# yzh503/vm-placement-migration-gym

Measured on AMD Instinct MI355X. Metric: env-steps/sec (batched) at 100-PM config, 1/2/4/8 GPUs; reward MAE vs CPU ref, higher is better.
Workload: dtype f64

## Files before the change

include/vmp.h:

```cpp
#ifndef VMP_H
#define VMP_H

#include <stdint.h>

#ifdef __cplusplus
extern "C" {
#endif

#define VMP_ABI_VERSION 14

#define VMP_OK 0
#define VMP_EINVAL (-1)
#define VMP_EDEVICE (-2)
#define VMP_EOOM (-3)
#define VMP_ESTATE (-4)

#define VMP_REWARD_WR 0
#define VMP_REWARD_UT 1
#define VMP_REWARD_KL 2
#define VMP_SEQ_UNIFORM 0
#define VMP_SEQ_LOWUNIFORM 1
#define VMP_SEQ_HIGHUNIFORM 2
#define VMP_REC_STEPS 0
#define VMP_REC_REWARD 1
// ... 196 lines not shown
int vmp_actor_head_bf16_sample(int32_t B, int32_t K, int32_t V, int32_t A, const uint16_t *h,
                               const uint16_t *weight, const float *bias,
                               const uint32_t *mask_bits, float wait_ratio, int32_t wait_index,
                               uint64_t seed, uint64_t offset, const uint64_t *rng_counter,
                               int32_t *action, float *logprob, float *entropy, float *workspace,
                               void *hip_stream);
int vmp_actor_head_bf16_bwd(int32_t B, int32_t K, int32_t V, int32_t A, const uint16_t *h,
                            const uint16_t *weight, const float *bias, const uint32_t *mask_bits,
                            const int32_t *action, const float *g_logprob,
                            const float *g_entropy, uint16_t *dlogits, int32_t ld, float *dbias,
                            float *workspace, void *hip_stream);
int64_t vmp_actor_head_bf16_bwd_workspace(int32_t B, int32_t V, int32_t A);

int vmp_record_enable(vmp_handle *h, int32_t on);
int vmp_record_read(vmp_handle *h, uint32_t *hist, double *sums);

int vmp_reqlog_enable(vmp_handle *h, int64_t capacity);
int vmp_reqlog_info(const vmp_handle *h, int64_t *capacity);
int vmp_reqlog_read(vmp_handle *h, int32_t *rows, int64_t *meta);

int vmp_series_enable(vmp_handle *h, int64_t capacity, int32_t stride, int32_t pm_rows);
int vmp_series_info(const vmp_handle *h, int64_t *capacity, int32_t *stride, int32_t *pm_rows);
int vmp_series_read(vmp_handle *h, double *rows, float *pm, int64_t *meta);

int vmp_debug_fail_alloc(int32_t n);
int64_t vmp_debug_live_allocs(void);

int vmp_debug_stamps(vmp_handle *h, uint64_t *out);

int vmp_debug_quiet_violations(int64_t *count);

int vmp_debug_occupancy(vmp_handle *h, int32_t *blocks_per_cu, int32_t *lds_bytes);

#ifdef __cplusplus
}
#endif
#endif
```

vm-placement-migration-gym_amd/csrc/vmp_capi.cpp:

```cpp
#include <hip/hip_runtime.h>

#include <cmath>
#include <cstdlib>
#include <cstring>
#include <string>
#include <vector>

#include "../../include/vmp.h"
#include "vmp_carve.h"
#include "vmp_host.h"
#include "vmp_kernels.h"
#include "vmp_layout.h"
#include "vmp_record.h"
#include "vmp_reqlog.h"
#include "vmp_series.h"
#include "vmp_trace.h"

using namespace vmp;

namespace vmp {
int policy_fail(int code, const char *msg) { return fail(code, msg); }
}

struct vmp_handle {
  vmp_config cfg;
  int32_t N, P, V, A, D, W32;
  int32_t device;
  int32_t eval_mode;
  hipStream_t stream;
  uint32_t *vmw;
  double *pm;
  EnvHdr *hdr;
  double *lg_arr, *lg_svc;
  PoisConst arr, svc;
  EnvParams prm;
  uint32_t *scratch_bits;
  PoisConst *pois_dev;
  uint64_t *stamps;
  uint64_t *jump_dev;
  uint8_t *bigscr;
  bool big;
  bool rec_on;
  RecArgs rec;
  int32_t *rec_act;
  uint8_t *rec_valid;
  double *rec_reward;
  bool rq_on;
  ReqArgs rq;
  bool sr_on;
  SerArgs sr;
  double *sr_reward;
  double *wl;
  PoisConst *wl_rec;
  PoisConst *pois_env;
  double *lg_shared;
  int32_t lg_shared_n;
  TraceDesc *tr_tab;
  uint64_t *tr_data;
  TraceDesc *tr_host;
  int32_t tr_n;
  int32_t *tr_map;
  int64_t *tr_info;
  uint64_t tr_hash;
};

namespace {

using EnvKernel = void (*)(EnvParams, StepOut);
template <int VPT>
EnvKernel env_kernel_tr(bool ext, bool one) {
  if (ext) return k_env_ext_tr<VPT>;
  return one ? k_env_tr<VPT, true> : k_env_tr<VPT, false>;
}
template <int VPT>
EnvKernel env_kernel(bool ext, bool one, bool wl, bool tr) {
  if (tr) return env_kernel_tr<VPT>(ext, one);
  if (ext) return wl ? k_env_ext<VPT, true> : k_env_ext<VPT, false>;
  if (one) return wl ? k_env<VPT, true, true> : k_env<VPT, true, false>;
  return wl ? k_env<VPT, false, true> : k_env<VPT, false, false>;
}

int launch_env(vmp_handle *h, const StepOut &o) {
  dim3 grid((h->N + kEnvWavesPerBlock - 1) / kEnvWavesPerBlock), block(64 * kEnvWavesPerBlock);
  EnvParams p = h->prm;
  const bool wl = h->pois_env != nullptr, tr = h->tr_tab != nullptr;
  const int spt = big_spt(h->V);
  p.scap = kSpecDraws;
  p.lds_wave_bytes = launch_wave_bytes(p, o.k_steps);
  const size_t lds = launch_lds(p, o.k_steps, h->big, spt);
  if (!lds_fits(lds, h->big)) return fail(VMP_EINVAL, "config too large for the LDS carve");
  if (h->big) {
    if (tr) launch_big_env_tr(spt, o.k_steps == 1, h->N, lds, h->stream, p, o);
    else if (wl) launch_big_env_wl(spt, o.k_steps == 1, h->N, lds, h->stream, p, o);
    else launch_big_env(spt, o.k_steps == 1, h->N, lds, h->stream, p, o);
    return launched();
  }
  if (o.actions && o.k_steps != 1) return fail(VMP_EINVAL, "external actions take one step per launch");
  const int need = (h->V + 63) / 64;
  const auto pick = need <= 1 ? env_kernel<1> : need <= 2 ? env_kernel<2> : need <= 4 ? env_kernel<4>
                    : need <= 8 ? env_kernel<8> : env_kernel<16>;
  hipLaunchKernelGGL(pick(o.actions != nullptr, o.k_steps == 1, wl, tr), grid, block, lds, h->stream, p, o);
  return launched();
}

StepOut empty_out() {
  StepOut o;
  std::memset(&o, 0, sizeof(o));
  o.policy = -1;
  return o;
}

void refresh_params(vmp_handle *h) {
  h->prm.eval_mode = h->eval_mode;
  h->prm.limit = h->eval_mode ? h->cfg.eval_steps : h->cfg.training_steps;
}

void scratch_free(vmp_handle *h) {
  dev_free(h->rec_act);
  dev_free(h->rec_valid);
  h->rec_act = nullptr;
  h->rec_valid = nullptr;
}

int record_init(vmp_handle *h, const uint8_t *env_mask) {
  size_t n = (size_t)h->N * h->V;
  if ((size_t)h->N * 2 * VMP_REC_BINS > n) n = (size_t)h->N * 2 * VMP_REC_BINS;
  if ((size_t)h->N * VMP_NREC > n) n = (size_t)h->N * VMP_NREC;
  hipLaunchKernelGGL(k_record_init, dim3((unsigned)((n + 255) / 256)), dim3(256), 0, h->stream,
                     h->prm, h->rec, env_mask);
  return launched();
// ... 59 lines not shown
    return fail(VMP_EINVAL, "vms must be in [1, 10240] on this build");
  if (cfg->reward_function < 0 || cfg->reward_function > 2)
    return fail(VMP_EINVAL, "Function does not exist: reward_function");
  if (cfg->sequence < 0 || cfg->sequence > 2) return fail(VMP_EINVAL, "unknown sequence");
  if (!(cfg->arrival_rate >= 0) || !(cfg->service_length >= 0))
    return fail(VMP_EINVAL, "arrival_rate and service_length must be >= 0");
  for (int32_t i = 0; i < n_env; i++)
    if (seeds[i] < 0) return fail(VMP_EINVAL, "seeds must be non-negative");
  HIP_TRY(hipSetDevice(device));
  vmp_handle *h = new vmp_handle();
  std::memset(h, 0, sizeof(*h));
  h->cfg = *cfg;
  h->N = n_env;
  h->P = cfg->pms;
  h->V = cfg->vms;
  h->A = cfg->allow_null_action ? cfg->pms + 2 : cfg->pms + 1;
  h->D = 3 * cfg->vms + 2 * cfg->pms;
  h->W32 = (h->A + 31) / 32;
  const char *force = getenv("VMP_BIG_KERNEL");
  h->big = cfg->vms > kMaxVPT * kWaveSize || (force && force[0] == '1');
  h->device = device;
  h->stream = nullptr;
  int rc = setup_pois(cfg->arrival_rate, h->arr, &h->lg_arr);
  if (rc == VMP_OK) rc = setup_pois(cfg->service_length, h->svc, &h->lg_svc);
  if (rc == VMP_OK) rc = create_rest(h, cfg, n_env, seeds);
  if (rc != VMP_OK) return fail_after(rc, [&] { vmp_destroy(h); });
  *out = h;
  return VMP_OK;
}

static int create_rest(vmp_handle *h, const vmp_config *cfg, int32_t n_env, const int64_t *seeds) {
  hipError_t e1 = dev_malloc(&h->vmw, sizeof(uint32_t) * (size_t)n_env * vm_pitch(h->V));
  hipError_t e2 = dev_malloc(&h->pm, sizeof(double) * (size_t)n_env * 2 * h->P);
  hipError_t e3 = dev_malloc(&h->hdr, sizeof(EnvHdr) * (size_t)n_env);
  if (e1 != hipSuccess || e2 != hipSuccess || e3 != hipSuccess)
    return fail(VMP_EOOM, "device allocation failed");
  HIP_TRY(hipMemset(h->hdr, 0, sizeof(EnvHdr) * (size_t)n_env));
  EnvParams &p = h->prm;
  p.N = h->N;
  p.P = h->P;
  p.V = h->V;
  p.A = h->A;
  p.D = h->D;
  p.W32 = h->W32;
  p.reward = cfg->reward_function;
  p.cap_target_util = cfg->cap_target_util;
  int64_t M = cfg->training_steps > cfg->eval_steps ? cfg->training_steps : cfg->eval_steps;
  p.M2 = 2 * M;
  p.beta = cfg->beta;
  p.seq_lo = cfg->sequence == VMP_SEQ_HIGHUNIFORM ? 0.25 : 0.1;
  double hi = cfg->sequence == VMP_SEQ_LOWUNIFORM ? 0.65 : 1.0;
  p.seq_range = hi - p.seq_lo;
  {
    PoisConst pc[2] = {h->arr, h->svc};
    HIP_TRY(dev_malloc(&h->pois_dev, sizeof(pc)));
    HIP_TRY(hipMemcpy(h->pois_dev, pc, sizeof(pc), hipMemcpyHostToDevice));
    p.pois = h->pois_dev;
    uint64_t jt[kJumpWords];
    pcg_jump_table(jt);
    HIP_TRY(dev_malloc(&h->jump_dev, sizeof(jt)));
    HIP_TRY(hipMemcpy(h->jump_dev, jt, sizeof(jt), hipMemcpyHostToDevice));
    p.jump = h->jump_dev;
  }
  p.vmw = h->vmw;
  p.pm = h->pm;
  p.hdr = h->hdr;
  if (h->big) carve_big(h->P, h->V, p);
  else carve_wave(h->P, h->V, p);
  if (h->big) {
    HIP_TRY(dev_malloc(&h->bigscr, (size_t)n_env * 4 * (size_t)h->V));
// ... 722 lines not shown
  SnapDesc d;
  HIP_TRY(hipStreamSynchronize(h->stream));
  HIP_TRY(hipMemcpy(&d, src, sizeof(d), hipMemcpyDeviceToHost));
  if (d.magic != kSnapMagic || d.abi != VMP_ABI_VERSION || d.hdr_bytes != (int32_t)sizeof(EnvHdr))
    return fail(VMP_EINVAL, "vmp_restore: not a snapshot of this library version");
  if (d.N != h->N || d.P != h->P || d.V != h->V || d.A != h->A || !same_config(d.cfg, h->cfg))
    return fail(VMP_EINVAL, "vmp_restore: snapshot of another env count or config");
  const uint8_t *s = (const uint8_t *)src;
  const SnapLayout l(h);
  if ((d.workload != 0) != (h->wl != nullptr))
    return fail(VMP_EINVAL, "vmp_restore: snapshot and handle differ in having a per-env workload");
  if ((d.traced != 0) != (h->tr_tab != nullptr))
    return fail(VMP_EINVAL, "vmp_restore: snapshot and handle differ in having a trace");
  if (h->tr_tab && d.trace_hash != h->tr_hash)
    return fail(VMP_EINVAL, "vmp_restore: snapshot of another trace");
  if (h->wl) {
    std::vector<double> w(2 * (size_t)h->N);
    HIP_TRY(hipMemcpy(w.data(), s + l.wl, l.nw, hipMemcpyDeviceToHost));
    if (std::memcmp(w.data(), h->wl, l.nw) != 0)
      return fail(VMP_EINVAL, "vmp_restore: snapshot of another per-env workload");
  }
  HIP_TRY(hipMemcpyAsync(h->hdr, s + l.hdr, l.nh, hipMemcpyDeviceToDevice, h->stream));
  HIP_TRY(hipMemcpyAsync(h->pm, s + l.pm, l.np, hipMemcpyDeviceToDevice, h->stream));
  HIP_TRY(hipMemcpyAsync(h->vmw, s + l.vmw, l.nv, hipMemcpyDeviceToDevice, h->stream));
  if (h->rec_on)
    if (const int rc = record_init(h, nullptr)) return rc;
  if (h->rq_on)
    if (const int rc = reqlog_init(h, nullptr)) return rc;
  return h->sr_on ? series_init(h, nullptr) : VMP_OK;
}

int64_t vmp_debug_live_allocs(void) { return g_live.load(); }

int vmp_debug_quiet_violations(int64_t *count) {
  if (!count) return fail(VMP_EINVAL, "null argument");
  const int64_t v = quiet_violations_take();
  if (v == -1) return fail(VMP_EINVAL, "library built without -DVMP_CHECK_QUIET");
  if (v < 0) return fail(VMP_EDEVICE, "vmp_debug_quiet_violations: device read failed");
  *count = v;
  return VMP_OK;
}

int vmp_debug_fail_alloc(int32_t n) {
  if (n < 0) return fail(VMP_EINVAL, "n must be >= 0");
  g_fail_alloc.store(n);
  return VMP_OK;
}

int vmp_debug_occupancy(vmp_handle *h, int32_t *blocks_per_cu, int32_t *lds_bytes) {
  if (!h || !blocks_per_cu || !lds_bytes) return fail(VMP_EINVAL, "null argument");
  if (!h->big) return fail(VMP_EINVAL, "occupancy query covers the block kernel (V > 1024) only");
  const int spt = big_spt(h->V);
  const size_t lds1 = launch_lds(h->prm, 1, true, spt);
  int st = 0;
  *blocks_per_cu = big_occupancy(spt, lds1, &st);
  *lds_bytes = (int32_t)lds1 + st;
  return VMP_OK;
}

int vmp_debug_stamps(vmp_handle *h, uint64_t *out) {
  if (!h || !out) return fail(VMP_EINVAL, "null argument");
  if (!h->stamps) return fail(VMP_EINVAL, "library built without -DVMP_STAMPS");
  HIP_TRY(hipMemcpyAsync(out, h->stamps, sizeof(uint64_t) * kStamps * (size_t)h->N,
                         hipMemcpyDeviceToDevice, h->stream));
  HIP_TRY(hipMemsetAsync(h->stamps, 0, sizeof(uint64_t) * kStamps * (size_t)h->N, h->stream));
  return VMP_OK;
// ... 4 lines not shown
```

vm-placement-migration-gym_amd/csrc/vmp_env_aux.h:

```cpp
#ifndef VMP_ENV_AUX_H
#define VMP_ENV_AUX_H

#include <hip/hip_runtime.h>
#include <stdint.h>

#include "vmp_dev.h"
#include "vmp_env_common.h"
#include "vmp_kernels.h"
#include "vmp_layout.h"
#include "vmp_np_rng.h"
#include "vmp_np_sum.h"

namespace vmp {

__global__ __launch_bounds__(256) void k_reset(EnvParams p, const int64_t *seeds,
                                               const uint8_t *env_mask, float *obs) {
  const int lane = lane_id();
  const int e = uni(blockIdx.x * kWavesPerBlock + (threadIdx.x >> 6));
  if (e >= p.N) return;
  if (env_mask && !env_mask[e]) return;
  EnvHdr *h = p.hdr + e;
  const int V = p.V, P = p.P;
  if (lane < 4) {
    Pcg r;
// ... 160 lines not shown
  __syncthreads();
  const int lane = lane_id(), e = blockIdx.x;
  const Lds L = make_lds(p, (char LDSP *)lds);
  const int V = p.V, P = p.P;
  const uint32_t *row = p.vmw + (int64_t)e * vm_pitch(V);
  int n_ex = 0;
  for (int b = 0; b < V; b += 64) {
    const int v = b + lane;
    const uint32_t w = v < V ? row[vm_slot_idx(v)] : (uint32_t)(P + 1);
    const bool ex = v < V && (int)(w & 0xFFFFu) <= P;
    const uint64_t m = ballot(ex);
    if (ex) {
      const int rk = n_ex + below(m, lane);
      L.ccomp[rk] = (uint8_t)((w >> 16) & 0xFFu);
      L.mcomp[rk] = (uint8_t)((w >> 24) & 0xFFu);
    }
    n_ex += __popcll(m);
  }
  wsync();
  const double *ct = cent;
  const uint8_t LDSP *cc = L.ccomp;
  const uint8_t LDSP *cm = L.mcomp;
  const double sc = wave_pw_sum(n_ex, [=](int i) { return ct[cc[i]]; }, L.pw);
  const double sm = wave_pw_sum(n_ex, [=](int i) { return ct[cm[i]]; }, L.pw);
  if (lane == 0) {
    double tcm = sc / (double)P, tmm = sm / (double)P;
    if (p.cap_target_util && tcm > 1) tcm = 1.0;
    if (p.cap_target_util && tmm > 1) tmm = 1.0;
    p.hdr[e].tcm = tcm;
    p.hdr[e].tmm = tmm;
  }
}

}

#endif
```

vm-placement-migration-gym_amd/csrc/vmp_env_wave.h:

```cpp
#ifndef VMP_ENV_WAVE_H
#define VMP_ENV_WAVE_H

#include <hip/hip_runtime.h>
#include <stdint.h>

#include "vmp_dev.h"
#include "vmp_env_common.h"
#include "vmp_kernels.h"
#include "vmp_layout.h"
#include "vmp_stamps.h"

namespace vmp {

template <int VPT>
__device__ __forceinline__ int64_t heuristic_apply(const EnvParams &p, const Lds &L,
                                                   const Tables &T, uint32_t (&wa)[VPT],
                                                   int policy, int32_t *act_out,
                                                   uint8_t *valid_out, bool quiet, int qkind,
                                                   bool &fit_any STAMP_PARAMS) {
  const int lane = lane_id();
  const int P = p.P, WAIT = p.P;
  const bool bf = policy == 1;
  uint32_t pend = 0;
#pragma unroll
  for (int s = 0; s < VPT; s++)
    if (w_pl(wa[s]) == WAIT) pend |= 1u << s;
  uint32_t won = 0, bad = 0;
  int64_t n_place = 0;
  fit_any = false;
#ifdef VMP_CHECK_QUIET
  if (ballot(pend != 0)) {
#else
  if (!quiet && ballot(pend != 0)) {
#endif
    for (int i = lane; i < P; i += 64) {
      const float fcv = (float)L.cpu[i], fmv = (float)L.mem[i];
      L.fcpu[i] = fcv;
      L.fmem[i] = fmv;
      L.tc[i] = (uint8_t)(fit_threshold(fcv) + 1);
      L.tm[i] = (uint8_t)(fit_threshold(fmv) + 1);
    }
// ... 422 lines not shown

template <int VPT>
__device__ __forceinline__ void write_mask(const EnvParams &p, const Lds &L, const Tables &T,
                                           const uint32_t (&wa)[VPT], uint32_t *bits) {
  const int lane = fresh_lane();
  const int P = p.P, A = p.A, W = p.W32, WAIT = p.P, NUL = p.P + 1;
#pragma unroll
  for (int s = 0; s < VPT; s++) {
    const int v = s * 64 + lane;
    const bool in = live(wa[s]);
    const int c = in ? w_pl(wa[s]) : NUL;
    const double vc = T.cent[w_cc(wa[s])], vm = T.cent[w_cm(wa[s])];
    const bool waiting = in && c == WAIT;
    const bool anyw = ballot(waiting) != 0;
#pragma unroll 1
    for (int w = 0; w < W; w++) {
      uint32_t word = 0xFFFFFFFFu;
      const int a0 = w * 32;
      if (c >= a0 && c < a0 + 32 && c < A) word &= ~(1u << (c - a0));
      if (c < P && WAIT >= a0 && WAIT < a0 + 32) word &= ~(1u << (WAIT - a0));
      if (anyw) {
        const int hi = min(a0 + 32, P);
#pragma unroll 1
        for (int q = a0; q < hi; q++) {
          const bool fit = (L.cpu[q] + vc <= 1) && (L.mem[q] + vm <= 1);
          if (waiting && fit) word &= ~(1u << (q - a0));
        }
      }
      if (in) bits[(int64_t)v * W + w] = word;
    }
  }
}

__device__ __forceinline__ bool idle_step(const EnvParams &p, const StepOut &o, const Lds &L) {
#ifdef VMP_CHECK_QUIET
  return false;
#else
  const uint64_t ph = L.hdr->pad;
  const uint32_t t32 = (uint32_t)L.hdr->timestep;
  const uint32_t nf = (uint32_t)ph;
  const bool q1 = (ph >> 62) & 1u, q2 = (ph >> 60) & 1u;
  const bool idle = o.k_steps == 1 && p.reward == 0 && !o.act_out && !o.valid && !o.mask_bits &&
                    2 * p.P <= 256 && (ph >> 63) && q1 != q2 &&
                    (ph & 0x0FFFFFFF00000000ull) == 0 && nf != 0u && (int32_t)(nf - t32) > 1;
  return uni((int)idle) != 0;
#endif
}

template <int VPT>
__device__ __forceinline__ void idle_body(const EnvParams &p, const StepOut &o, const Lds &L,
                                          const float LDSP *fcent, int e,
                                          const uint32_t (&wa)[VPT]) {
  const int lane = lane_id();
  const int V = p.V;
  EnvHdr LDSP *H = L.hdr;
  const int64_t a = L.arr[0];
  const uint64_t ph = H->pad;
  const int64_t ts = H->timestep;
  const bool term = ts >= p.limit;
  if (lane == 0) {
    if (o.reward) gptr(o.reward)[e] = ((ph >> 61) & 1u) ? -H->waiting_ratio : 0.0;
    if (o.done) gptr(o.done)[e] = (uint8_t)term;
    if (o.done_count) gptr(o.done_count)[e] += (int64_t)term;
  }
  if (o.obs) {
    float *obs = o.obs + (int64_t)e * p.D;
#pragma unroll
    for (int s = 0; s < VPT; s++) {
      const int v = s * 64 + lane;
      if (live(wa[s])) {
        ST_NT(obs + v, (float)w_pl(wa[s]));
        ST_NT(obs + V + v, fcent[w_cc(wa[s])]);
        ST_NT(obs + 2 * V + v, fcent[w_cm(wa[s])]);
      }
    }
    for (int i = lane; i < 2 * p.P; i += 64) ST_NT(obs + 3 * V + i, (float)L.cpu[i]);
  }
  wsync();
  if (lane == 0) {
    H->timestep = ts + 1;
    H->total_requests += a;
    H->dropped += a;
  }
  wsync();
  if (lane < 32)
    gptr(reinterpret_cast<uint64_t *>(p.hdr + e))[lane] = reinterpret_cast<uint64_t LDSP *>(H)[lane];
}

template <int VPT, bool ONE, bool EXT, int SRC>
__device__ __forceinline__ void env_body(const EnvParams &p, const StepOut &o) {
  extern __shared__ __align__(16) char lds[];
  __shared__ Tables T;
#ifdef VMP_STAMPS
  const uint64_t t_start = __builtin_amdgcn_s_memtime();
  const uint64_t rt_start = __builtin_amdgcn_s_memrealtime();
#endif
  const int lane = lane_id();
  const int wid = threadIdx.x >> 6;
  const int e_raw = uni(blockIdx.x * kEnvWavesPerBlock + wid);
  const int e = e_raw < p.N ? e_raw : p.N - 1;
  char LDSP *base = (char LDSP *)lds + wid * p.lds_wave_bytes;
  const Lds L = make_lds(p, base);
  const int V = p.V, P = p.P;
  __builtin_amdgcn_s_setprio(2);
  const uint64_t hv = gptr(reinterpret_cast<const uint64_t *>(p.hdr + e))[lane & 31];
  static_assert(kEnvWavesPerBlock == 1, "Tables::pois holds one env's Poisson constants");
  constexpr int kPoisWords = (int)(2 * sizeof(PoisConst) / 4);
  uint32_t pw = 0;
  if constexpr (SRC != kSrcTrace)
    pw = gptr(reinterpret_cast<const uint32_t *>(env_pois<SRC>(p, e)))[threadIdx.x % kPoisWords];
  TraceDesc td{nullptr, nullptr, 0, 0};
  if constexpr (SRC == kSrcTrace) td = env_trace(p, e);
  U128 JA{0, 0}, JM{0, 0};
  if (SRC != kSrcTrace && o.k_steps > 0) {
    const uint64_t GLBP *jt = gptr(p.jump + 4 * lane);
    JA = U128{jt[0], jt[1]};
    JM = U128{jt[2], jt[3]};
  }
  const double *pm = p.pm + (int64_t)e * 2 * P;
  const int n_pm = 2 * P;
  double pv[4];
#pragma unroll
  for (int j = 0; j < 4; j++) pv[j] = pm[min(j * 64 + lane, n_pm - 1)];
  __asm__ volatile("" ::: "memory");
  const uint32_t GLBP *vlo = gptr(p.vmw + (int64_t)e * vm_pitch(V));
  uint32_t wa[VPT], rem[VPT];
#pragma unroll
  for (int s = 0; s < VPT; s++) {
    const int v = s * 64 + lane;
    const uint32_t x = vlo[vw_row(s, lane)];
    wa[s] = v < V ? x : (uint32_t)kPad;
    if (ONE) {
      rem[s] = 0;
    } else {
      const uint32_t y = vlo[vw_row(s, lane) + 64];
      rem[s] = v < V ? y : 0u;
    }
  }
// ... 16 lines not shown
#pragma unroll
    for (int j = 0; j < 4; j++)
      if (j * 64 + lane < n_pm) L.cpu[j * 64 + lane] = pv[j];
  }
  if constexpr (SRC == kSrcTrace) {
    if (o.k_steps > 0) trace_preload(L, td, o.k_steps);
  } else {
    if (o.k_steps > 0) predraw(p, L, T, o.k_steps, V, JA, JM);
  }
#ifdef VMP_STAMPS
  const uint64_t t_drawn = __builtin_amdgcn_s_memtime();
#endif
  if (!EXT) {
#pragma unroll
    for (int j = 0; j < 4; j++)
      if (j * 64 + lane < n_pm) L.cpu[j * 64 + lane] = pv[j];
  }
  for (int i = 256 + lane; i < n_pm; i += 64) L.cpu[i] = pm[i];
  for (int i = lane; i < (n_pm + 63) / 64; i += 64) L.pdirty[i] = 0;
  wsync();
#ifdef VMP_STAMPS
  __shared__ uint64_t st_lds[kEnvWavesPerBlock * kStamps];
#endif
  STAMP_DECL_AT((uint64_t LDSP *)st_lds + wid * kStamps)
#ifdef VMP_STAMPS
  if (lane == 0) {
    st_acc[13] = t_loaded - t_start;
    st_acc[14] = t_drawn - t_loaded;
    st_acc[15] = st_prev - t_drawn;
  }
#endif
  if constexpr (ONE && !EXT && SRC != kSrcTrace) {
  if (idle_step(p, o, L)) {
    idle_body<VPT>(p, o, L, (const float LDSP *)T.fcent, e, wa);
#ifdef VMP_STAMPS
    if (p.stamps && lane == 0) stamp_idle(p.stamps + (int64_t)e * kStamps, t_start, rt_start);
#endif
    return;
  }
  }
  bool term = false;
  int64_t ndone = 0;
  uint32_t dirty = 0;
  uint32_t fb = 0;
  uint32_t hiv[VPT];
  uint32_t nf = 0u;
  bool want_nf = false;
  bool skip_time = false;
  uint32_t nf_carry = 0u;
  if (ONE && !EXT) {
#ifndef VMP_CHECK_QUIET
    const uint64_t ph = L.hdr->pad;
    nf_carry = (uint32_t)ph;
    const bool skip_h = ((ph >> 62) & 1u) || (((ph >> 60) & 1u) && !o.act_out && !o.valid);
    skip_time = skip_h && (ph >> 63) && ((ph >> 32) & 1u) == 0u && nf_carry != 0u &&
                (int32_t)(nf_carry - (uint32_t)L.hdr->timestep) > 1;
#endif
    const uint32_t GLBP *hb = vlo + 64 + (skip_time ? 0 : lane);
    const int hs = skip_time ? 0 : 128;
#pragma unroll
    for (int s = 0; s < VPT; s++) hiv[s] = hb[s * hs];
    __asm__ volatile("" ::: "memory");
  }
  uint32_t *vmo = p.vmw + (int64_t)e * vm_pitch(V);
  const int k_steps = ONE ? 1 : o.k_steps;
  int qkind = EXT ? 0 : (((L.hdr->pad >> 62) & 1u) ? 1 : (((L.hdr->pad >> 60) & 1u) ? 2 : 0));
  bool has_ex = (L.hdr->pad >> 61) & 1u;
// ... 83 lines not shown
          ST_NT(vmo + iw, wa[s]);
          ST_NT(vmo + iw + 64, rem[s]);
        } else if (w_pl(wa[s]) == P + 1) {
          ST_NT(vmo + iw, wa[s]);
          ST_NT(vmo + iw + 64, 0u);
        } else {
          uint32_t GLBP *w32 = gptr(vmo);
          w32[iw] = wa[s];
          __hip_atomic_fetch_add(w32 + iw + 64, w_pl(wa[s]) < P ? t32 : 0u - t32,
                                 __ATOMIC_RELAXED, __HIP_MEMORY_SCOPE_AGENT);
        }
      }
    }
    double *pmo = p.pm + (int64_t)e * 2 * P;
    for (int i = lane, j = 0; i < 2 * P; i += 64, j++)
      if ((L.pdirty[j] >> lane) & 1ull) ST_NT(pmo + i, (double)L.cpu[i]);
    {
      uint64_t hint = 0;
      if (ONE) {
        bool anynull = false;
#pragma unroll
        for (int s = 0; s < VPT; s++) anynull |= w_pl(wa[s]) == P + 1;
        uint32_t m = nf;
        const bool nn = ballot(anynull) != 0;
        if (!nn && want_nf) {
#pragma unroll
          for (int o = 32; o > 0; o >>= 1) m = min(m, (uint32_t)__shfl_xor((int)m, o));
        }
        hint = (1ull << 63) | ((uint64_t)nn << 32) | m;
      }
      hint |= ((uint64_t)(qkind == 1) << 62) | ((uint64_t)(qkind == 2) << 60) |
              ((uint64_t)has_ex << 61);
      wsync();
      if (lane == 0) L.hdr->pad = hint;
      wsync();
    }
    if (lane < 32)
      gptr(reinterpret_cast<uint64_t *>(p.hdr + e))[lane] = reinterpret_cast<uint64_t LDSP *>(L.hdr)[lane];
  }
  STAMP(6);
#ifdef VMP_STAMPS
  if (lane == 0) {
    st_acc[7] = (__builtin_amdgcn_s_memrealtime() - rt_start) * 1000;
    st_acc[9] = __builtin_amdgcn_s_memtime() - t_start;
  }
#endif
  STAMP_FLUSH();
}

template <int VPT, bool ONE, bool WL>
__global__ __launch_bounds__(64 * kEnvWavesPerBlock, ONE ? VMP_WAVES_PER_EU_ONE : VMP_WAVES_PER_EU) void k_env(EnvParams p, StepOut o) {
  env_body<VPT, ONE, false, WL ? kSrcEnv : kSrcConfig>(p, o);
}
template <int VPT, bool WL>
__global__ __launch_bounds__(64 * kEnvWavesPerBlock, VPT == 1 ? 4 : VMP_WAVES_PER_EU_ONE) void k_env_ext(EnvParams p, StepOut o) {
  env_body<VPT, true, true, WL ? kSrcEnv : kSrcConfig>(p, o);
}
template <int VPT, bool ONE>
__global__ __launch_bounds__(64 * kEnvWavesPerBlock, ONE ? VMP_WAVES_PER_EU_ONE : VMP_WAVES_PER_EU) void k_env_tr(EnvParams p, StepOut o) {
  env_body<VPT, ONE, false, kSrcTrace>(p, o);
}
template <int VPT>
__global__ __launch_bounds__(64 * kEnvWavesPerBlock, VPT == 1 ? 4 : VMP_WAVES_PER_EU_ONE) void k_env_ext_tr(EnvParams p, StepOut o) {
  env_body<VPT, true, true, kSrcTrace>(p, o);
}

#ifdef VMP_ENV_TR
// ... 40 lines not shown
```

vm-placement-migration-gym_amd/csrc/vmp_kernels.h:

```cpp
#ifndef VMP_KERNELS_H
#define VMP_KERNELS_H

#include <hip/hip_runtime.h>
#include <stdint.h>

#include "vmp_carve.h"
#include "vmp_layout.h"

namespace vmp {

constexpr int kStamps = 24;

template <int VPT, bool ONE, bool WL = false>
__global__ void k_env(EnvParams p, StepOut o);
template <int VPT, bool WL = false>
__global__ void k_env_ext(EnvParams p, StepOut o);
template <int VPT, bool ONE>
__global__ void k_env_tr(EnvParams p, StepOut o);
template <int VPT>
__global__ void k_env_ext_tr(EnvParams p, StepOut o);
__global__ void k_rank(EnvParams p, int64_t *rank);
__global__ void k_target_means_lds(EnvParams p);
__global__ void k_reset(EnvParams p, const int64_t *seeds, const uint8_t *env_mask, float *obs);
__global__ void k_export(EnvParams p, int64_t *placement, double *vm_cpu, double *vm_mem,
                         double *cpu, double *mem, int64_t *remaining, int64_t *rank);
__global__ void k_counters(EnvParams p, int64_t *ctr, double *st);
__global__ void k_target_means(EnvParams p);
__global__ void k_mask_bool(int64_t rows, int A, int W, const uint32_t *bits, uint8_t *mask);
__global__ void k_act_obs(int P, int V, int policy, const float *obs, int32_t *act);

void launch_big_env(int spt, bool one, int n_env, size_t lds, hipStream_t s, const EnvParams &p,
                    const StepOut &o);
void launch_big_env_wl(int spt, bool one, int n_env, size_t lds, hipStream_t s,
                       const EnvParams &p, const StepOut &o);
void launch_big_env_tr(int spt, bool one, int n_env, size_t lds, hipStream_t s,
                       const EnvParams &p, const StepOut &o);
int big_occupancy(int spt, size_t lds, int *static_lds);

int64_t quiet_violations_take();

}

#endif
```

vm-placement-migration-gym_amd/vmp/_lib.py:

```python
import ctypes
import os

_HERE = os.path.dirname(os.path.abspath(__file__))
LIB_PATH = os.environ.get("VMP_LIB_PATH") or os.path.join(_HERE, "libvmp.so")

REWARDS = {"wr": 0, "ut": 1, "kl": 2}
SEQUENCES = {"uniform": 0, "lowuniform": 1, "highuniform": 2}
POLICIES = {"firstfit": 0, "bestfit": 1}

EXPORTS = (
    "vmp_abi_version", "vmp_last_error", "vmp_create", "vmp_destroy", "vmp_set_stream",
    "vmp_set_eval", "vmp_dims", "vmp_set_workload", "vmp_get_workload", "vmp_set_trace",
    "vmp_clear_trace", "vmp_trace_info", "vmp_reset", "vmp_step",
    "vmp_heuristic_act", "vmp_heuristic_act_obs",
    "vmp_heuristic_step", "vmp_rollout_heuristic", "vmp_mask", "vmp_mask_bool", "vmp_get_obs",
    "vmp_get_counters", "vmp_get_stats", "vmp_get_state", "vmp_get_rank", "vmp_gae",
    "vmp_policy_head", "vmp_policy_head_backward", "vmp_policy_head_backward_bf16",
    "vmp_actor_head", "vmp_actor_head_bf16_fwd", "vmp_actor_head_bf16_sample",
    "vmp_actor_head_bf16_bwd",
    "vmp_actor_head_bf16_bwd_workspace", "vmp_actor_mlp_packed_floats", "vmp_actor_mlp_pack",
    "vmp_actor_mlp_f32", "vmp_actor_mlp_head_f32", "vmp_step_mask", "vmp_record_enable",
    "vmp_record_read", "vmp_reqlog_enable", "vmp_reqlog_info", "vmp_reqlog_read",
    "vmp_series_enable", "vmp_series_info", "vmp_series_read",
    "vmp_snapshot_bytes", "vmp_snapshot", "vmp_restore",
    "vmp_debug_fail_alloc", "vmp_debug_live_allocs", "vmp_debug_stamps", "vmp_debug_occupancy",
    "vmp_debug_quiet_violations",
)


class VmpConfig(ctypes.Structure):
    _fields_ = [("arrival_rate", ctypes.c_double), ("service_length", ctypes.c_double),
                ("pms", ctypes.c_int32), ("vms", ctypes.c_int32),
                ("training_steps", ctypes.c_int64), ("eval_steps", ctypes.c_int64),
                ("seed", ctypes.c_int64), ("reward_function", ctypes.c_int32),
                ("sequence", ctypes.c_int32), ("cap_target_util", ctypes.c_int32),
                ("allow_null_action", ctypes.c_int32), ("beta", ctypes.c_double)]


class VmpTrace(ctypes.Structure):
    _fields_ = [("steps", ctypes.c_int64), ("offs", ctypes.c_void_p), ("cpu", ctypes.c_void_p),
                ("mem", ctypes.c_void_p), ("runtime", ctypes.c_void_p)]


def to_c_config(cfg):
    if cfg.reward_function not in REWARDS:
        raise ValueError(f"Function does not exist: {cfg.reward_function}")
    if cfg.sequence not in SEQUENCES:
        raise AttributeError(f"unknown sequence {cfg.sequence!r}")
    return VmpConfig(float(cfg.arrival_rate), float(cfg.service_length), int(cfg.pms),
                     int(cfg.vms), int(cfg.training_steps), int(cfg.eval_steps), int(cfg.seed),
                     REWARDS[cfg.reward_function], SEQUENCES[cfg.sequence],
                     int(bool(cfg.cap_target_util)), int(bool(cfg.allow_null_action)),
                     float(cfg.beta))


class VmpError(RuntimeError):
    pass


# ... 41 lines not shown
        "vmp_policy_head": (ctypes.c_int, [i32, i32, i32, i32, P, P, f32, i32, u64, u64, P, P, P,
                                            P, P, P]),
        "vmp_policy_head_backward": (ctypes.c_int, [i32, i32, i32, P, P, P, P, P, P, P]),
        "vmp_policy_head_backward_bf16": (ctypes.c_int, [i32, i32, i32, P, P, P, P, P, P, P]),
        "vmp_actor_head": (ctypes.c_int, [i32, i32, i32, i32, i32, P, P, P, P, f32, i32, u64, u64,
                                           P, P, P, P, P, P, P]),
        "vmp_actor_head_bf16_fwd": (ctypes.c_int, [i32, i32, i32, i32, P, P, P, P, P, P, P, P, P]),
        "vmp_actor_head_bf16_sample": (ctypes.c_int, [i32, i32, i32, i32, P, P, P, P, f32, i32,
                                                       u64, u64, P, P, P, P, P, P]),
        "vmp_actor_head_bf16_bwd": (ctypes.c_int, [i32, i32, i32, i32, P, P, P, P, P, P, P, P,
                                                    i32, P, P, P]),
        "vmp_actor_head_bf16_bwd_workspace": (ctypes.c_int64, [i32, i32, i32]),
        "vmp_actor_mlp_packed_floats": (ctypes.c_int64, [i32, i32, i32, i32]),
        "vmp_actor_mlp_pack": (ctypes.c_int, [i32, i32, i32, i32, P, P, P, P, P]),
        "vmp_actor_mlp_f32": (ctypes.c_int, [i32, i32, i32, i32, i32, P, P, P, P, P, P, P]),
        "vmp_actor_mlp_head_f32": (ctypes.c_int, [i32, i32, i32, i32, i32, i32, P, P, P, P, P, P,
                                                   f32, i32, u64, u64, P, i32, P, P, P, P, P]),
        "vmp_record_enable": (ctypes.c_int, [P, i32]),
        "vmp_record_read": (ctypes.c_int, [P, P, P]),
        "vmp_reqlog_enable": (ctypes.c_int, [P, i64]),
        "vmp_reqlog_info": (ctypes.c_int, [P, P]),
        "vmp_reqlog_read": (ctypes.c_int, [P, P, P]),
        "vmp_series_enable": (ctypes.c_int, [P, i64, i32, i32]),
        "vmp_series_info": (ctypes.c_int, [P, P, P, P]),
        "vmp_series_read": (ctypes.c_int, [P, P, P, P]),
        "vmp_snapshot_bytes": (ctypes.c_int, [P, P]),
        "vmp_snapshot": (ctypes.c_int, [P, P]),
        "vmp_restore": (ctypes.c_int, [P, P]),
        "vmp_debug_fail_alloc": (ctypes.c_int, [i32]),
        "vmp_debug_live_allocs": (ctypes.c_int64, []),
        "vmp_debug_stamps": (ctypes.c_int, [P, P]),
        "vmp_debug_occupancy": (ctypes.c_int, [P, P, P]),
        "vmp_debug_quiet_violations": (ctypes.c_int, [P]),
    }
    for name, (res, args) in sig.items():
        f = getattr(L, name, None)
        if f is None and name.startswith("vmp_debug_"):
            continue
        if f is None:
            raise VmpError(f"libvmp lacks {name}")
        f.restype, f.argtypes = res, args
    if L.vmp_abi_version() != 14:
        raise VmpError("libvmp ABI mismatch")
    _lib = L
    return L


def check(rc):
    if rc != 0:
        raise VmpError(f"libvmp error {rc}: {lib().vmp_last_error().decode()}")
    return rc


def ptr(t):
    return None if t is None else ctypes.c_void_p(t.data_ptr())
```

Before: 254.9 million.

## Reorder single-step env launch so idle envs run last, alternating direction

For single-step launches of the wave-per-env kernel, each launch now reverses block-to-env order on alternate calls. It also swaps busy envs from the late tail of each 64-env chunk with idle envs from the early head, using per-env idle flags written in the previous step into a double-buffered area after the headers. The aim is to cut tail imbalance: idle fast-path envs get scheduled last so expensive envs start early. The cost is an extra flag read plus ballot in tail blocks, a flag store per step, and a larger header allocation. Env-to-block mapping becomes stateful across launches, which risks mismatches with snapshot or restore.

```diff
diff --git a/include/vmp.h b/include/vmp.h
--- a/include/vmp.h
+++ b/include/vmp.h
@@ -252,6 +252,9 @@
 
 int vmp_debug_occupancy(vmp_handle *h, int32_t *blocks_per_cu, int32_t *lds_bytes);
 
+int vmp_debug_launch_order(vmp_handle *h, int32_t mode);
+int vmp_debug_launch_map(vmp_handle *h, int32_t *env_of_block, uint8_t *flags_read);
+
 #ifdef __cplusplus
 }
 #endif
diff --git a/vm-placement-migration-gym_amd/csrc/vmp_capi.cpp b/vm-placement-migration-gym_amd/csrc/vmp_capi.cpp
--- a/vm-placement-migration-gym_amd/csrc/vmp_capi.cpp
+++ b/vm-placement-migration-gym_amd/csrc/vmp_capi.cpp
@@ -10,6 +10,7 @@
 #include "vmp_carve.h"
 #include "vmp_host.h"
 #include "vmp_kernels.h"
+#include "vmp_launch_order.h"
 #include "vmp_layout.h"
 #include "vmp_record.h"
 #include "vmp_reqlog.h"
@@ -62,6 +63,8 @@
   int32_t *tr_map;
   int64_t *tr_info;
   uint64_t tr_hash;
+  uint32_t lo_count;
+  int32_t lo_mode, lo_div;
 };
 
 namespace {
@@ -78,6 +81,10 @@
   if (ext) return wl ? k_env_ext<VPT, true> : k_env_ext<VPT, false>;
   if (one) return wl ? k_env<VPT, true, true> : k_env<VPT, true, false>;
   return wl ? k_env<VPT, false, true> : k_env<VPT, false, false>;
+}
+
+uint32_t launch_order_word(const vmp_handle *h) {
+  return lo_word(h->lo_mode, (int)(h->lo_count & 1u), h->N, lo_tail(h->N, h->lo_div));
 }
 
 int launch_env(vmp_handle *h, const StepOut &o) {
@@ -96,6 +103,10 @@
     return launched();
   }
   if (o.actions && o.k_steps != 1) return fail(VMP_EINVAL, "external actions take one step per launch");
+  if (o.k_steps == 1) {
+    p.pad0 = (int32_t)launch_order_word(h);
+    h->lo_count++;
+  }
   const int need = (h->V + 63) / 64;
   const auto pick = need <= 1 ? env_kernel<1> : need <= 2 ? env_kernel<2> : need <= 4 ? env_kernel<4>
                     : need <= 8 ? env_kernel<8> : env_kernel<16>;
@@ -221,10 +232,17 @@
 static int create_rest(vmp_handle *h, const vmp_config *cfg, int32_t n_env, const int64_t *seeds) {
   hipError_t e1 = dev_malloc(&h->vmw, sizeof(uint32_t) * (size_t)n_env * vm_pitch(h->V));
   hipError_t e2 = dev_malloc(&h->pm, sizeof(double) * (size_t)n_env * 2 * h->P);
-  hipError_t e3 = dev_malloc(&h->hdr, sizeof(EnvHdr) * (size_t)n_env);
+  const size_t hdr_bytes = sizeof(EnvHdr) * (size_t)n_env + 2 * (size_t)lo_flag_bytes(n_env);
+  hipError_t e3 = dev_malloc(&h->hdr, hdr_bytes);
   if (e1 != hipSuccess || e2 != hipSuccess || e3 != hipSuccess)
     return fail(VMP_EOOM, "device allocation failed");
-  HIP_TRY(hipMemset(h->hdr, 0, sizeof(EnvHdr) * (size_t)n_env));
+  HIP_TRY(hipMemset(h->hdr, 0, hdr_bytes));
+  h->lo_mode = kLoDefaultMode;
+  h->lo_div = kLoDefaultDiv;
+  if (const char *m = getenv("VMP_LAUNCH_ORDER")) {
+    if (m[0] >= '0' && m[0] <= '2') h->lo_mode = m[0] - '0';
+    if (m[0] && m[1] == ':' && atoi(m + 2) >= 4) h->lo_div = atoi(m + 2);
+  }
   EnvParams &p = h->prm;
   p.N = h->N;
   p.P = h->P;
@@ -1013,6 +1031,26 @@
 
 int64_t vmp_debug_live_allocs(void) { return g_live.load(); }
 
+int vmp_debug_launch_order(vmp_handle *h, int32_t mode) {
+  if (!h) return fail(VMP_EINVAL, "null handle");
+  if (mode < kLoIndex || mode > kLoIdleLast) return fail(VMP_EINVAL, "launch order mode must be 0, 1 or 2");
+  h->lo_mode = mode;
+  return VMP_OK;
+}
+
+int vmp_debug_launch_map(vmp_handle *h, int32_t *env_of_block, uint8_t *flags_read) {
+  if (!h || !env_of_block || !flags_read) return fail(VMP_EINVAL, "null argument");
+  if (h->big) return fail(VMP_EINVAL, "the block kernel (V > 1024) keeps index order");
+  EnvParams p = h->prm;
+  p.pad0 = (int32_t)launch_order_word(h);
+  hipLaunchKernelGGL(k_launch_map, dim3(h->N), dim3(64), 0, h->stream, p, env_of_block);
+  if (const int rc = launched()) return rc;
+  const size_t nb = (size_t)lo_flag_bytes(h->N);
+  const uint8_t *flags = reinterpret_cast<const uint8_t *>(h->hdr + h->N) + nb * (h->lo_count & 1u);
+  HIP_TRY(hipMemcpyAsync(flags_read, flags, nb, hipMemcpyDeviceToDevice, h->stream));
+  return VMP_OK;
+}
+
 int vmp_debug_quiet_violations(int64_t *count) {
   if (!count) return fail(VMP_EINVAL, "null argument");
   const int64_t v = quiet_violations_take();
diff --git a/vm-placement-migration-gym_amd/csrc/vmp_env_aux.h b/vm-placement-migration-gym_amd/csrc/vmp_env_aux.h
--- a/vm-placement-migration-gym_amd/csrc/vmp_env_aux.h
+++ b/vm-placement-migration-gym_amd/csrc/vmp_env_aux.h
@@ -216,6 +216,12 @@
   }
 }
 
+__global__ __launch_bounds__(64) void k_launch_map(EnvParams p, int32_t *env_of_block) {
+  int fidx;
+  const int e = uni(lo_swap_env(p, lo_position((uint32_t)p.pad0, p.N, (int)blockIdx.x), fidx));
+  if (lane_id() == 0) env_of_block[blockIdx.x] = e;
+}
+
 }
 
 #endif
diff --git a/vm-placement-migration-gym_amd/csrc/vmp_env_wave.h b/vm-placement-migration-gym_amd/csrc/vmp_env_wave.h
--- a/vm-placement-migration-gym_amd/csrc/vmp_env_wave.h
+++ b/vm-placement-migration-gym_amd/csrc/vmp_env_wave.h
@@ -7,6 +7,7 @@
 #include "vmp_dev.h"
 #include "vmp_env_common.h"
 #include "vmp_kernels.h"
+#include "vmp_launch_order.h"
 #include "vmp_layout.h"
 #include "vmp_stamps.h"
 
@@ -495,6 +496,38 @@
   }
 }
 
+__device__ __forceinline__ uint8_t *lo_flags(const EnvParams &p, int parity) {
+  return reinterpret_cast<uint8_t *>(p.hdr + p.N) + (int64_t)parity * lo_flag_bytes(p.N);
+}
+__device__ __forceinline__ int lo_swap_env(const EnvParams &p, int q, int &fidx) {
+  const uint32_t w = (uint32_t)p.pad0;
+  fidx = -1;
+  if (lo_mode(w) == kLoIdleLast) {
+    const int C = lo_chunks(p.N), T = lo_T(w), nr = lo_nr(w);
+    int r = q / C;
+    const int c = q - r * C;
+    if (lo_in_tail(r, T, nr)) {
+      const int lane = lane_id();
+      const uint8_t GLBP *line = gptr(lo_flags(p, lo_parity(w))) + (int64_t)c * kLoChunk;
+      const bool in = lane < 2 * T;
+      const uint8_t f = in ? line[lo_lane_rank(lane, T, nr)] : (uint8_t)0;
+      const uint32_t busy = (uint32_t)ballot(in && f != 0);
+      r = uni(lo_partner(busy, T, nr, lo_parity(w), r));
+      q = r * C + c;
+    }
+    fidx = c * kLoChunk + r;
+  }
+  return q;
+}
+__device__ __forceinline__ void lo_store_flag(const EnvParams &p, int fidx, uint64_t ph, int64_t t) {
+  if (fidx < 0) return;
+  const uint32_t nf = (uint32_t)ph;
+  const bool q1 = (ph >> 62) & 1u, q2 = (ph >> 60) & 1u;
+  const bool idle = (ph >> 63) && q1 != q2 && (ph & 0x0FFFFFFF00000000ull) == 0 && nf != 0u &&
+                    (int32_t)(nf - (uint32_t)t) > 1;
+  gptr(lo_flags(p, lo_parity((uint32_t)p.pad0) ^ 1))[fidx] = (uint8_t)!idle;
+}
+
 __device__ __forceinline__ bool idle_step(const EnvParams &p, const StepOut &o, const Lds &L) {
 #ifdef VMP_CHECK_QUIET
   return false;
@@ -513,7 +546,7 @@
 template <int VPT>
 __device__ __forceinline__ void idle_body(const EnvParams &p, const StepOut &o, const Lds &L,
                                           const float LDSP *fcent, int e,
-                                          const uint32_t (&wa)[VPT]) {
+                                          const uint32_t (&wa)[VPT], int fidx) {
   const int lane = lane_id();
   const int V = p.V;
   EnvHdr LDSP *H = L.hdr;
@@ -544,6 +577,7 @@
     H->timestep = ts + 1;
     H->total_requests += a;
     H->dropped += a;
+    lo_store_flag(p, fidx, ph, ts + 1);
   }
   wsync();
   if (lane < 32)
@@ -560,13 +594,22 @@
 #endif
   const int lane = lane_id();
   const int wid = threadIdx.x >> 6;
-  const int e_raw = uni(blockIdx.x * kEnvWavesPerBlock + wid);
-  const int e = e_raw < p.N ? e_raw : p.N - 1;
+  int fidx = -1;
+  int e_raw = uni(blockIdx.x * kEnvWavesPerBlock + wid);
+  if constexpr (ONE) e_raw = uni(lo_position((uint32_t)p.pad0, p.N, e_raw));
+  int e = e_raw < p.N ? e_raw : p.N - 1;
   char LDSP *base = (char LDSP *)lds + wid * p.lds_wave_bytes;
   const Lds L = make_lds(p, base);
   const int V = p.V, P = p.P;
   __builtin_amdgcn_s_setprio(2);
-  const uint64_t hv = gptr(reinterpret_cast<const uint64_t *>(p.hdr + e))[lane & 31];
+  uint64_t hv = gptr(reinterpret_cast<const uint64_t *>(p.hdr + e))[lane & 31];
+  if constexpr (ONE && !EXT && SRC != kSrcTrace) {
+    const int e2 = uni(lo_swap_env(p, e, fidx));
+    if (e2 != e) {
+      e = e_raw = e2;
+      hv = gptr(reinterpret_cast<const uint64_t *>(p.hdr + e))[lane & 31];
+    }
+  }
   static_assert(kEnvWavesPerBlock == 1, "Tables::pois holds one env's Poisson constants");
   constexpr int kPoisWords = (int)(2 * sizeof(PoisConst) / 4);
   uint32_t pw = 0;
@@ -649,7 +692,7 @@
 #endif
   if constexpr (ONE && !EXT && SRC != kSrcTrace) {
   if (idle_step(p, o, L)) {
-    idle_body<VPT>(p, o, L, (const float LDSP *)T.fcent, e, wa);
+    idle_body<VPT>(p, o, L, (const float LDSP *)T.fcent, e, wa, fidx);
 #ifdef VMP_STAMPS
     if (p.stamps && lane == 0) stamp_idle(p.stamps + (int64_t)e * kStamps, t_start, rt_start);
 #endif
@@ -799,7 +842,10 @@
       hint |= ((uint64_t)(qkind == 1) << 62) | ((uint64_t)(qkind == 2) << 60) |
               ((uint64_t)has_ex << 61);
       wsync();
-      if (lane == 0) L.hdr->pad = hint;
+      if (lane == 0) {
+        L.hdr->pad = hint;
+        if constexpr (ONE && !EXT && SRC != kSrcTrace) lo_store_flag(p, fidx, hint, L.hdr->timestep);
+      }
       wsync();
     }
     if (lane < 32)
diff --git a/vm-placement-migration-gym_amd/csrc/vmp_kernels.h b/vm-placement-migration-gym_amd/csrc/vmp_kernels.h
--- a/vm-placement-migration-gym_amd/csrc/vmp_kernels.h
+++ b/vm-placement-migration-gym_amd/csrc/vmp_kernels.h
@@ -28,6 +28,7 @@
 __global__ void k_target_means(EnvParams p);
 __global__ void k_mask_bool(int64_t rows, int A, int W, const uint32_t *bits, uint8_t *mask);
 __global__ void k_act_obs(int P, int V, int policy, const float *obs, int32_t *act);
+__global__ void k_launch_map(EnvParams p, int32_t *env_of_block);
 
 void launch_big_env(int spt, bool one, int n_env, size_t lds, hipStream_t s, const EnvParams &p,
                     const StepOut &o);
diff --git a/vm-placement-migration-gym_amd/csrc/vmp_launch_order.h b/vm-placement-migration-gym_amd/csrc/vmp_launch_order.h
--- /dev/null
+++ b/vm-placement-migration-gym_amd/csrc/vmp_launch_order.h
@@ -0,0 +1,89 @@
+#ifndef VMP_LAUNCH_ORDER_H
+#define VMP_LAUNCH_ORDER_H
+
+#include <stdint.h>
+
+#if defined(__HIPCC__) || defined(__CUDACC__)
+#define VMP_LO_HD __host__ __device__
+#else
+#define VMP_LO_HD
+#endif
+
+namespace vmp {
+
+constexpr int kLoIndex = 0, kLoDirection = 1, kLoIdleLast = 2;
+constexpr int kLoChunk = 64;
+constexpr int kLoDefaultMode = kLoIdleLast;
+constexpr int kLoDefaultDiv = 4;
+
+VMP_LO_HD inline int lo_chunks(int N) { return (N + kLoChunk - 1) / kLoChunk; }
+VMP_LO_HD inline int lo_ranks(int N) { return N / lo_chunks(N); }
+VMP_LO_HD inline int lo_tail(int N, int div) {
+  const int nr = lo_ranks(N);
+  return (nr < 8 || div <= 0) ? 0 : nr / div;
+}
+VMP_LO_HD inline uint32_t lo_word(int mode, int parity, int N, int T) {
+  if (mode == kLoIndex) return 0u;
+  return (uint32_t)(parity & 1) | ((uint32_t)mode << 1) | ((uint32_t)T << 8) |
+         ((uint32_t)lo_ranks(N) << 16);
+}
+VMP_LO_HD inline int lo_parity(uint32_t w) { return (int)(w & 1u); }
+VMP_LO_HD inline int lo_mode(uint32_t w) { return (int)((w >> 1) & 3u); }
+VMP_LO_HD inline int lo_T(uint32_t w) { return (int)((w >> 8) & 0xFFu); }
+VMP_LO_HD inline int lo_nr(uint32_t w) { return (int)((w >> 16) & 0xFFu); }
+VMP_LO_HD inline int64_t lo_flag_bytes(int N) { return (int64_t)kLoChunk * lo_chunks(N); }
+
+VMP_LO_HD inline int lo_position(uint32_t w, int N, int b) { return lo_parity(w) ? N - 1 - b : b; }
+
+VMP_LO_HD inline bool lo_in_tail(int r, int T, int nr) { return r < nr && (r < T || r >= nr - T); }
+VMP_LO_HD inline int lo_lane_rank(int i, int T, int nr) { return i < T ? i : nr - 2 * T + i; }
+
+VMP_LO_HD inline int lo_kth_bit(uint32_t m, int k) {
+  for (; k > 0; k--) m &= m - 1u;
+  return __builtin_ctz(m);
+}
+
+VMP_LO_HD inline int lo_partner(uint32_t busy, int T, int nr, int parity, int r) {
+  const uint32_t ends = (1u << T) - 1u;
+  const uint32_t lo = busy & ends, hi = (busy >> T) & ends;
+  const uint32_t A = parity ? lo : hi;
+  const uint32_t B = (parity ? ~hi : ~lo) & ends;
+  const int base_lo = 0, base_hi = nr - T;
+  const bool r_low = r < T;
+  const int j = r_low ? r : r - base_hi;
+  const bool late = r_low == (parity != 0);
+  const uint32_t mine = late ? A : B, other = late ? B : A;
+  if (!((mine >> j) & 1u)) return r;
+  const int k = __builtin_popcount(mine & ((1u << j) - 1u));
+  if (k >= __builtin_popcount(other)) return r;
+  return (r_low ? base_hi : base_lo) + lo_kth_bit(other, k);
+}
+
+VMP_LO_HD inline int lo_env_of_position(uint32_t w, int N, int q, const uint8_t *flags) {
+  if (lo_mode(w) != kLoIdleLast || !flags) return q;
+  const int C = lo_chunks(N), T = lo_T(w), nr = lo_nr(w);
+  const int r = q / C, c = q - r * C;
+  if (!lo_in_tail(r, T, nr)) return q;
+  uint32_t busy = 0;
+  for (int i = 0; i < 2 * T; i++)
+    busy |= (uint32_t)(flags[(int64_t)c * kLoChunk + lo_lane_rank(i, T, nr)] != 0) << i;
+  return lo_partner(busy, T, nr, lo_parity(w), r) * C + c;
+}
+
+VMP_LO_HD inline void lo_ref_chunk(const uint8_t *line, int T, int nr, int parity, int *map) {
+  int A[kLoChunk], B[kLoChunk], na = 0, nb = 0;
+  for (int r = 0; r < nr; r++) map[r] = r;
+  const int late0 = parity ? 0 : nr - T, early0 = parity ? nr - T : 0;
+  for (int i = 0; i < T; i++) {
+    if (line[late0 + i] != 0) A[na++] = late0 + i;
+    if (line[early0 + i] == 0) B[nb++] = early0 + i;
+  }
+  for (int k = 0; k < na && k < nb; k++) {
+    map[A[k]] = B[k];
+    map[B[k]] = A[k];
+  }
+}
+
+}
+
+#endif
diff --git a/vm-placement-migration-gym_amd/vmp/_lib.py b/vm-placement-migration-gym_amd/vmp/_lib.py
--- a/vm-placement-migration-gym_amd/vmp/_lib.py
+++ b/vm-placement-migration-gym_amd/vmp/_lib.py
@@ -24,7 +24,7 @@
     "vmp_series_enable", "vmp_series_info", "vmp_series_read",
     "vmp_snapshot_bytes", "vmp_snapshot", "vmp_restore",
     "vmp_debug_fail_alloc", "vmp_debug_live_allocs", "vmp_debug_stamps", "vmp_debug_occupancy",
-    "vmp_debug_quiet_violations",
+    "vmp_debug_quiet_violations", "vmp_debug_launch_order", "vmp_debug_launch_map",
 )
 
 
@@ -132,6 +132,8 @@
         "vmp_debug_stamps": (ctypes.c_int, [P, P]),
         "vmp_debug_occupancy": (ctypes.c_int, [P, P, P]),
         "vmp_debug_quiet_violations": (ctypes.c_int, [P]),
+        "vmp_debug_launch_order": (ctypes.c_int, [P, i32]),
+        "vmp_debug_launch_map": (ctypes.c_int, [P, P, P]),
     }
     for name, (res, args) in sig.items():
         f = getattr(L, name, None)
```

Measured after the change: 271.6 million (median of 6 runs). 1.07x the previous value.
